# ielym/fastvision

Hardware: AMD Instinct MI355X
Metric: images/sec (640×640, bs=32/GPU) YOLOv3 train step, 1/2/4/8 MI355X (higher is better)
Workload: dtype bf16

## Files before the change

fastvision_amd/_lib.py:

```python
import ctypes as C
import os

HERE = os.path.dirname(os.path.abspath(__file__))
LIB_PATH = os.path.join(HERE, 'csrc', 'libfastvision_amd.so')
if os.environ.get('FVA_LIB_PATH'):
    if os.environ.get('FVA_EXPERIMENTS') == '1':
        LIB_PATH = os.environ['FVA_LIB_PATH']
        import sys
        print(f'fastvision_amd: EXPERIMENT -- loading {LIB_PATH} instead of the in-tree library (FVA_LIB_PATH)', file=sys.stderr)
    else:
        raise RuntimeError('fastvision_amd: FVA_LIB_PATH is set but FVA_EXPERIMENTS=1 is not -- refusing to load another library silently')

F32, BF16 = 0, 1


class ConvDesc(C.Structure):
    _fields_ = [(n, C.c_int32) for n in ('dtype', 'B', 'H', 'W', 'Cin', 'Cout', 'ksize', 'stride', 'in_pad', 'dy_pad')]


class HeadLevel(C.Structure):
    _fields_ = [('data', C.c_void_p), ('grad', C.c_void_p),
                ('sb', C.c_int64), ('sa', C.c_int64), ('sy', C.c_int64), ('sx', C.c_int64), ('sk', C.c_int64),
                ('B', C.c_int32), ('A', C.c_int32), ('H', C.c_int32), ('W', C.c_int32), ('K', C.c_int32),
                ('anchor_w', C.c_float * 8), ('anchor_h', C.c_float * 8), ('stride', C.c_float)]
# ... 53 lines not shown
    'fva_side_stream_renew': (_I, []),
    'fva_conv_debug_stamps': (_I, [_P, _I]),
    'fva_conv_patch_kernel': (_I, [_I]),
    'fva_profile_stop': (_I, [_P, _P, _P, _I]),
    'fva_conv_pack_weights': (_I, [_D, _P, _P, _P, _P]),
    'fva_conv_packed_elems': (_L, [_D, _I]),
    'fva_conv_pack_weights_multi': (_I, [_P, _I, _L, _P]),
    'fva_conv_pack_weights_tiled': (_I, [_P, _I, _I, _P]),
    'fva_conv_last_kernel': (C.c_char_p, []),
    'fva_conv_fwd': (_I, [_D, _P, _P, _P, _P, _P]),
    'fva_conv1x1_fwd_apply': (_I, [_D, _P, _P, _P, _P, _I, _P, _P, _P, _P, _P]),
    'fva_conv_fwd_acc': (_I, [_D, _P, _P, _P, _P, _I, _P]),
    'fva_bn_acc_finalize': (_I, [C.POINTER(BnFwdAcc), _L, _I, _P]),
    'fva_bn_silu_apply_acc': (_I, [_I, _P, C.POINTER(BnFwdAcc), _P, _I, _P, _I, _I, _I, _I, _I, _P]),
    'fva_conv1x1_fwd_apply_acc': (_I, [_D, _P, C.POINTER(BnFwdAcc), _P, _I, _P, _P, _P, _P, _I, _P]),
    'fva_conv_fwd_bnact': (_I, [_D, _P, _P, _P, _P, _P, _P, _I, _P]),
    'fva_conv_stat_blocks': (_I, [_D]),
    'fva_conv_dgrad': (_I, [_D, _P, _P, _P, _P, _P]),
    'fva_conv_dgrad_bnstats': (_I, [_D, _P, _P, _P, _P, C.POINTER(BnBwdFuse), _P]),
    'fva_conv_dgrad_stat_rows': (_I, [_D]),
    'fva_conv_wgrad': (_I, [_D, _P, _P, _P, _I, _P, _L, _P]),
    'fva_conv_wgrad_workspace': (_L, [_D]),
    'fva_conv_wgrad_plan': (_I, [_I]),
    'fva_stem_fwd': (_I, [_I, _P, _P, _P, _P, _P, _L, _I, _I, _I, _I, _I, _P]),
    'fva_stem_fwd_workspace': (_L, [_I, _I, _I, _I]),
    'fva_stem_stat_blocks': (_I, [_I, _I, _I, _I]),
    'fva_stem_fused_blocks': (_I, [_I, _I, _I]),
    'fva_stem_wgrad': (_I, [_I, _P, _P, _P, _I, _P, _L, _I, _I, _I, _I, _I, _P]),
    'fva_stem_wgrad_workspace': (_L, [_I, _I, _I, _I, _I]),
    'fva_stem_wgrad_mfma': (_I, [_P, _P, _P, _P, _L, _I, _I, _I, _P]),
    'fva_stem_wgrad_mfma_workspace': (_L, []),
    'fva_stem_pack': (_I, [_P, _P, _L, _I, _I, _I, _I, _P]),
    'fva_stem_fused': (_I, [_I, _P, _P, _P, _P, _P, _P, _P, _P, _P, _P, _I, _I, _I, _I, _P]),
    'fva_head_fwd': (_I, [_D, _P, _P, _P, _P, _P]),
    'fva_head_bwd_prepare': (_I, [_I, _P, _P, _P, _P, _I, _P, _I, _I, _I, _I, _I, _P]),
    'fva_bn_finalize': (_I, [_P, _I, _I, _L, _I, _P, _P, _P, _P, _P, _F, _F, _P, _P, _P, _P, _P]),
    'fva_bn_partial_rows': (_I, [_I]),
    'fva_bn_eval_coeffs': (_I, [_I, _P, _P, _P, _P, _F, _P, _P, _P]),
    'fva_bn_silu_apply': (_I, [_I, _P, _P, _P, _P, _I, _P, _I, _I, _I, _I, _I, _P]),
    'fva_bn_silu_bwd_reduce': (_I, [_I, _P, _P, _P, _P, _P, _P, _P, _I, _L, _I, _P]),
    'fva_bn_silu_bwd_reduce_acc': (_I, [_I, _P, _P, _P, _P, _P, _P, _P, _I, _L, _I, _P]),
    'fva_bn_bwd_blocks': (_I, [_I, _L, _I]),
    'fva_bn_bwd_finalize': (_I, [_P, _I, _I, _L, _I, _P, _P, _P, _P, _I, _P, _P]),
    'fva_bn_silu_bwd_apply': (_I, [_I, _P, _P, _P, _P, _P, _P, _P, _P, _I, _I, _I, _I, _I, _P]),
    'fva_bn_silu_bwd_apply_acc': (_I, [_I, _P, _P, _P, _P, _P, _P, C.POINTER(BnBwdAcc), _P, _I, _I, _I, _I, _I, _P]),
    'fva_upsample2_concat_fwd': (_I, [_I, _P, _I, _P, _I, _P, _I, _I, _I, _I, _I, _I, _P]),
    'fva_upsample2_concat_bwd': (_I, [_I, _P, _P, _P, _I, _I, _I, _I, _I, _I, _P]),
    'fva_pack_nchw': (_I, [_I, _P, _I, _L, _L, _L, _L, _P, _I, _I, _I, _I, _I, _P]),
    'fva_cast_nhwc': (_I, [_P, _I, _I, _P, _I, _I, _I, _I, _I, _I, _P]),
    'fva_yolov3_match': (_I, [_P, _I, _H, C.POINTER(MatchOut), _P]),
    'fva_yolov3_loss': (_I, [_P, _I, _H, _I, _F, _F, _F, _P, _P, _L, _P]),
    'fva_yolov3_loss_workspace': (_L, [_I, _H, _I]),
    'fva_yolov3_loss_dp': (_I, [_P, _I, _H, _I, _F, _F, _F, _P, _I, _P, _P, _L, _P]),
    'fva_scale_by_device_scalar': (_I, [_P, _L, _P, _P]),
    'fva_bce_loss': (_I, [_P, _P, _P, _P, _L, _L, _I, _I, _I, _P, _P, _P, _P]),
    'fva_row_loss': (_I, [_P, _P, _I, _I, _I, _F, _P, _P, _P, _P]),
    'fva_smooth_l1': (_I, [_P, _P, _L, _P, _P, _P, _P]),
    'fva_rows_relu_bwd_rows': (_I, [_I]),
    'fva_rows_relu_bwd': (_I, [_I, _P, _P, _P, _L, _P, _I, _I, _I, _P]),
    'fva_demo_loss': (_I, [_P, _I, _H, _I, _P, _P, _L, _P]),
    'fva_demo_loss_workspace': (_L, [_I, _H, _I]),
    'fva_demo_ciou_loss': (_I, [_P, _I, _H, _I, _P, _P, _L, _P]),
    'fva_demo_ciou_loss_workspace': (_L, [_I, _H, _I]),
    'fva_scale_head_groups': (_I, [_H, _P, _P, _P, _P]),
    'fva_iou_pairwise': (_I, [_I, _I, _I, _P, _P, _P, _P, _L, _F, _P]),
    'fva_iou_batch': (_I, [_I, _I, _I, _P, _P, _P, _L, _L, _F, _P]),
# ... 21 lines not shown
    'fva_colsum_scratch_rows': (_I, [_I]),
    'fva_colsum': (_I, [_P, _I, _I, _P, _P, _P]),
    'fva_maxpool2_fwd': (_I, [_I, _P, _I, _P, _I, _I, _I, _I, _I, _P]),
    'fva_maxpool2_bwd': (_I, [_I, _P, _P, _I, _P, _I, _I, _I, _I, _P]),
    'fva_rpn_decode': (_I, [_P, _P, _P, _P, _I, _I, _I, _I, _P]),
    'fva_rpn_match': (_I, [_P, _I, _P, _I, _I, _I, _I, _F, _F, _P, _P, _P]),
    'fva_fast_match': (_I, [_P, _I, _P, _I, _I, _F, _F, _F, _P, _P]),
    'fva_roi_align_fwd': (_I, [_I, _P, _I, _P, _I, _P, _I, _I, _I, _I, _I, _I, _F, _I, _P]),
    'fva_roi_align_bwd': (_I, [_P, _P, _I, _P, _I, _I, _I, _I, _I, _I, _F, _I, _P]),
    'fva_nms_select': (_I, [_P, _P, _I, _I, _I, C.POINTER(NmsParams), _P, _L, _P, _P, _P, _P]),
    'fva_gap_fwd': (_I, [_I, _P, _I, _I, _I, _I, _I, _P, _P]),
    'fva_gap_bwd': (_I, [_I, _P, _I, _I, _I, _I, _P, _P]),
    'fva_softmax_ce_workspace': (_L, [_I]),
    'fva_softmax_ce': (_I, [_P, _P, _I, _P, _I, _I, _I, _P, _P, _P, _P]),
    'fva_top1_accuracy': (_I, [_P, _I, _P, _I, _I, _I, _P, _P, _P]),
    'fva_bn_relu_apply': (_I, [_I, _P, _P, _P, _P, _I, _I, _I, _I, _I, _P]),
    'fva_bn_relu_bwd_reduce': (_I, [_I, _P, _P, _P, _P, _P, _P, _P, _I, _L, _I, _P]),
    'fva_bn_relu_bwd_apply': (_I, [_I, _P, _P, _P, _P, _P, _P, _P, _P, _I, _I, _I, _I, _I, _P]),
    'fva_bn_bias_running_mean': (_I, [_I, _P, _P, _F, _P]),
    'fva_bn_eval_coeffs_bias': (_I, [_I, _P, _P, _P, _P, _P, _F, _P, _P, _P]),
    'fva_adaptive_avgpool7_fwd': (_I, [_I, _P, _I, _I, _I, _I, _I, _P, _P]),
    'fva_adaptive_avgpool7_bwd': (_I, [_I, _P, _I, _I, _I, _I, _P, _P]),
    'fva_dropout_fwd': (_I, [_I, _P, _P, _L, _F, _P, _P]),
    'fva_dropout_bwd': (_I, [_I, _P, _P, _P, _L, _F, _P]),
    'fva_bn_frozen_bwd_blocks': (_I, [_I, _I, _I, _I, _I, _I]),
    'fva_bn_silu_frozen_bwd': (_I, [_I, _P, _P, _P, _P, _P, _P, _P, _P, _I, _I, _I, _I, _I, _P]),
    'fva_bn_relu_frozen_bwd': (_I, [_I, _P, _P, _P, _P, _P, _P, _P, _P, _I, _I, _I, _I, _I, _P]),
    'fva_bn_frozen_bwd_finalize': (_I, [_P, _I, _I, _I, _P, _P, _P, _P, _P]),
    'fva_bn_frozen_stats': (_I, [_I, _P, _P, _P, _F, _P, _P, _P]),
}
LABEL_I64, LABEL_F32 = 0, 1
REDUCE_MEAN, REDUCE_SUM = 0, 1
UNCHECKED = {'fva_conv_patch_kernel', 'fva_sgd_chunk_elems', 'fva_ema_chunk_elems', 'fva_rows_relu_bwd_rows', 'fva_colour_workspace', 'fva_conv_dgrad_stat_rows', 'fva_bias_relu_bwd_rows', 'fva_colsum_scratch_rows', 'fva_last_error', 'fva_version', 'fva_profile_stop', 'fva_conv_last_kernel', 'fva_conv_packed_elems', 'fva_conv_stat_blocks', 'fva_conv_wgrad_workspace', 'fva_conv_wgrad_plan',
             'fva_stem_stat_blocks', 'fva_stem_fused_blocks', 'fva_stem_wgrad_workspace', 'fva_stem_fwd_workspace', 'fva_stem_wgrad_mfma_workspace', 'fva_bn_bwd_blocks', 'fva_bn_partial_rows', 'fva_yolov3_loss_workspace',
             'fva_demo_loss_workspace', 'fva_demo_ciou_loss_workspace', 'fva_nms_candidates_workspace', 'fva_nms_select_workspace', 'fva_softmax_ce_workspace', 'fva_bn_frozen_bwd_blocks'}

_lib = None


def load():
    global _lib
    if _lib is not None:
        return _lib
    if not os.path.exists(LIB_PATH):
        raise RuntimeError(f'fastvision_amd: {LIB_PATH} is missing -- the HIP extension is REQUIRED (no CPU fallback). '
                           'Build it with `python fastvision_amd/csrc/build.py`.')
    lib = C.CDLL(LIB_PATH)
    for name, (res, args) in PROTOTYPES.items():
        fn = getattr(lib, name)
        fn.restype, fn.argtypes = res, args
    _lib = lib
    return lib


tracer = None


_fns = {}


def call(name, *args):
    fn = _fns.get(name)
    if fn is None:
        fn = _fns[name] = getattr(load(), name)
    lib = _lib
    if tracer is not None:
        span = tracer(name, args)
# ... 11 lines not shown
```

fastvision_amd/csrc/errors.hip:

```cpp
#include "common.h"
thread_local char fva_err_buf[512] = "";
extern "C" const char* fva_last_error(void) { return fva_err_buf; }
extern "C" int fva_version(void) { return 7; }
static thread_local const char* g_last_kernel = "";
void fva_note_kernel(const char* name) { g_last_kernel = name; }
extern "C" const char* fva_conv_last_kernel(void) { return g_last_kernel; }

#include <vector>
namespace {
struct Span { hipEvent_t e0, e1; int cls; double flop; };
std::vector<Span> g_spans;
int g_used = 0;
bool g_on = false;
unsigned g_mask = ~0u;
int g_stride = 1, g_seen = 0;
}

FvaProfileSpan::FvaProfileSpan(int cls, double flop, hipStream_t s) : slot(-1), stream(s) {
    if (!g_on || !((g_mask >> (cls & 0xff)) & 1u) || (g_seen++ % g_stride) != 0 || g_used >= (int)g_spans.size()) return;
    slot = g_used++;
    g_spans[slot].cls = cls;
    g_spans[slot].flop = flop;
    (void)hipEventRecord(g_spans[slot].e0, stream);
}
FvaProfileSpan::~FvaProfileSpan() {
    if (slot >= 0) (void)hipEventRecord(g_spans[slot].e1, stream);
}

extern "C" int fva_profile_start(int32_t max_spans) {
    if (max_spans < 0) return fva_fail(FVA_ERR_ARG, "fva_profile_start: negative span count");
    while ((int)g_spans.size() < max_spans) {
        Span sp{};
        if (hipEventCreate(&sp.e0) != hipSuccess || hipEventCreate(&sp.e1) != hipSuccess) return fva_fail(FVA_ERR_LAUNCH, "fva_profile_start: hipEventCreate failed");
        (void)hipEventRecord(sp.e0, nullptr);
        (void)hipEventRecord(sp.e1, nullptr);
        g_spans.push_back(sp);
// ... 123 lines not shown
```

fastvision_amd/csrc/stem.hip:

```cpp
#include <stdlib.h>

#include "common.h"

namespace {

constexpr int CO = 32;
constexpr int MAXJ = 36;

template <typename T>
__global__ __launch_bounds__(256) void stem_fwd_kernel(const float* __restrict__ img, const float* __restrict__ w,
                                                       T* __restrict__ y, float* __restrict__ stats, int B, int Cin, int H,
                                                       int W, int64_t M) {
    __shared__ float sw[MAXJ * CO];
    __shared__ float tile[256 * 33];
    const int tid = threadIdx.x;
    const int J = Cin * 9;
    for (int i = tid; i < J * CO; i += 256) {
        const int co = i % CO, j = i / CO;
        sw[j * CO + co] = w[co * J + j];
    }
    __syncthreads();
    const int64_t m = (int64_t)blockIdx.x * 256 + tid;
    const bool live = m < M;
    float acc[CO];
#pragma unroll
    for (int c = 0; c < CO; ++c) acc[c] = 0.f;
    if (live) {
        const int x = (int)(m % W), yy = (int)((m / W) % H), b = (int)(m / ((int64_t)W * H));
#pragma unroll 1
        for (int ci = 0; ci < Cin; ++ci) {
            const float* plane = img + ((int64_t)b * Cin + ci) * H * W;
#pragma unroll 1
            for (int kh = 0; kh < 3; ++kh)
// ... 218 lines not shown
        for (int c = 0; c < 2; ++c) {
            bf16x4 o;
#pragma unroll
            for (int j = 0; j < 4; ++j) {
                o[j] = (bf16_t)acc[c][j];
                s1[c][j] += acc[c][j];
                s2[c][j] += acc[c][j] * acc[c][j];
            }
            *(bf16x4*)(yo + 16 * c) = o;
        }
    }
    if (stats == nullptr) return;
#pragma unroll
    for (int c = 0; c < 2; ++c)
#pragma unroll
        for (int j = 0; j < 4; ++j) {
#pragma unroll
            for (int o = 1; o < 16; o <<= 1) {
                s1[c][j] += __shfl_xor(s1[c][j], o);
                s2[c][j] += __shfl_xor(s2[c][j], o);
            }
            if (r == 0) {
                red[0][wv][16 * c + 4 * g + j] = s1[c][j];
                red[1][wv][16 * c + 4 * g + j] = s2[c][j];
            }
        }
    __syncthreads();
    if (tid < 64) {
        const int which = tid >> 5, ch = tid & 31;
        stats[((int64_t)blockIdx.x * 2 + which) * 32 + ch] = (red[which][0][ch] + red[which][1][ch]) + (red[which][2][ch] + red[which][3][ch]);
    }
}

enum { STEM_STATS = 0, STEM_APPLY = 1, STEM_REDUCE = 2, STEM_DGRAD = 3 };

struct StemFusedParams {
    const uint2* img4;
    const float* w;
    const bf16_t* dz;
    const float *scale, *shift, *mean, *rstd, *coef;
    bf16_t* out;
    float* part;
    int Cin, H, W;
    int64_t M;
};

template <int MODE>
__global__ __launch_bounds__(256) void stem_fused_kernel(const StemFusedParams p) {
    __shared__ float red[2][4][32];
    const int tid = threadIdx.x, lane = tid & 63, wv = tid >> 6;
    const int r = lane & 15, g = lane >> 4;
    const int H = p.H, W = p.W, Wp = W + 2;
    __shared__ float wsh[CO * 27];
    bf16x8 wa[2][2];
    stem_weight_fragments<true>(p.w, p.Cin, wsh, wa);
    const int ta = 2 * g, tb = 2 * g + 1;
    const int offa = (ta / 3) * Wp + ta % 3, offb = (tb / 3) * Wp + tb % 3, offc = 2 * Wp + 2;
    float sc[2][4], sh[2][4], mu[2][4], rs[2][4], ka[2][4], k1[2][4], k2[2][4], s1[2][4], s2[2][4];
#pragma unroll
    for (int c = 0; c < 2; ++c)
#pragma unroll
        for (int j = 0; j < 4; ++j) {
            const int ch = 8 * g + 4 * c + j;
            s1[c][j] = s2[c][j] = 0.f;
            if constexpr (MODE != STEM_STATS) {
                sc[c][j] = p.scale[ch];
                sh[c][j] = p.shift[ch];
            }
            if constexpr (MODE == STEM_REDUCE || MODE == STEM_DGRAD) {
                mu[c][j] = p.mean[ch];
                rs[c][j] = p.rstd[ch];
            }
            if constexpr (MODE == STEM_DGRAD) {
                ka[c][j] = p.coef[ch];
                k1[c][j] = p.coef[32 + ch] * rs[c][j];
                k2[c][j] = p.coef[64 + ch] - k1[c][j] * mu[c][j];
            }
        }

    constexpr int STEM_NB = MODE == STEM_REDUCE ? 2 : 4;
    const int tiles_per_row = W / 16;
    const int nchunks = (int)((p.M / 16 + STEM_TPW - 1) / STEM_TPW);
    const int wvu = __builtin_amdgcn_readfirstlane(wv);
    for (int chunk = blockIdx.x * 4 + wvu; chunk < nchunks; chunk += gridDim.x * 4) {
    const int tile0 = chunk * STEM_TPW;
    int64_t m0 = (int64_t)tile0 * 16;
    const int row0 = tile0 / tiles_per_row;
    int x0 = (tile0 - row0 * tiles_per_row) * 16;
    const int b0 = row0 / H;
    int yy = row0 - b0 * H;
    int64_t hpix = ((int64_t)b0 * (H + 2) + yy) * Wp + x0;
    for (int bt = 0; bt < STEM_TPW / STEM_NB; ++bt) {
    uint2 la[STEM_NB], lb[STEM_NB], lc[STEM_NB];
    bf16x8 gz[STEM_NB];
    int64_t hp[STEM_NB];
    bool ok[STEM_NB];
#pragma unroll
    for (int i = 0; i < STEM_NB; ++i) {
        ok[i] = m0 < p.M;
        hp[i] = hpix + r;
        if (ok[i]) {
            const uint2* base = p.img4 + hp[i];
            la[i] = base[offa];
            lb[i] = base[offb];
            lc[i] = base[offc];
            if constexpr (MODE == STEM_REDUCE || MODE == STEM_DGRAD) gz[i] = *(const bf16x8*)(p.dz + (m0 + r) * 32 + 8 * g);
        }
        m0 += 16;
        x0 += 16;
        hpix += 16;
        if (x0 == W) {
// ... 36 lines not shown
                    const float du = (float)gzc[4 * c + j] * silu_grad(yv * sc[c][j] + sh[c][j]);
                    if constexpr (MODE == STEM_REDUCE) {
                        s1[c][j] += du;
                        s2[c][j] += du * (yv - mu[c][j]) * rs[c][j];
                    } else {
                        o[4 * c + j] = (bf16_t)(ka[c][j] * du + k1[c][j] * yv + k2[c][j]);
                    }
                }
            }
        }
        if constexpr (MODE == STEM_APPLY || MODE == STEM_DGRAD) *(bf16x8*)oo = o;
    }
    }
    }
    if constexpr (MODE == STEM_STATS || MODE == STEM_REDUCE) {
#pragma unroll
        for (int c = 0; c < 2; ++c)
#pragma unroll
            for (int j = 0; j < 4; ++j) {
#pragma unroll
                for (int o = 1; o < 16; o <<= 1) {
                    s1[c][j] += __shfl_xor(s1[c][j], o);
                    s2[c][j] += __shfl_xor(s2[c][j], o);
                }
                if (r == 0) {
                    red[0][wv][8 * g + 4 * c + j] = s1[c][j];
                    red[1][wv][8 * g + 4 * c + j] = s2[c][j];
                }
            }
        __syncthreads();
        if (tid < 64) {
            const int which = tid >> 5, ch = tid & 31;
            p.part[((int64_t)blockIdx.x * 2 + which) * 32 + ch] = (red[which][0][ch] + red[which][1][ch]) + (red[which][2][ch] + red[which][3][ch]);
        }
    }
}

constexpr int WGRAD_BLOCKS = 1024;
constexpr int STEM_FUSED_GRID = 2048;

}

extern "C" {

static bool stem_mfma(int dtype, int W) {
    static const bool on = [] { const char* e = getenv("FVA_STEM_MFMA"); return !e || atoi(e) != 0; }();
    return on && dtype == FVA_BF16 && W % 16 == 0;
}

int32_t fva_stem_stat_blocks(int dtype, int B, int H, int W) {
    const int64_t M = (int64_t)B * H * W;
    return stem_mfma(dtype, W) ? cdiv(M, STEM_BLOCK_PIX) : cdiv(M, 256);
}

int64_t fva_stem_fwd_workspace(int dtype, int B, int H, int W) {
    return stem_mfma(dtype, W) ? (int64_t)B * (H + 2) * (W + 2) * 8 + 64 : 0;
}

int fva_stem_fwd(int dtype, const float* img, const float* w, void* y, float* stats, void* workspace, int64_t workspace_bytes, int B,
                 int Cin, int H, int W, int Cout, void* stream) {
    if (!img || !w || !y) return fva_fail(FVA_ERR_ARG, "fva_stem_fwd: null pointer");
    if (Cout != CO || Cin < 1 || Cin > 3) return fva_fail(FVA_ERR_ARG, "fva_stem_fwd: needs Cout==32, Cin<=3 (got %d, %d)", Cout, Cin);
    const int64_t M = (int64_t)B * H * W;
    const int grid = cdiv(M, 256);
    hipStream_t s = (hipStream_t)stream;
    if (stem_mfma(dtype, W)) {
// ... 58 lines not shown
    hipLaunchKernelGGL(stem_pack_kernel, dim3((int)((hp + 255) / 256 < 65536 ? (hp + 255) / 256 : 65536)), dim3(256), 0, (hipStream_t)stream, img,
                       (uint2*)img4, B, Cin, H, W);
    FVA_LAUNCH_CHECK("stem_pack_kernel");
    return FVA_OK;
}

int fva_stem_fused(int mode, const void* img4, const float* w, const void* dz, const float* scale, const float* shift, const float* mean,
                   const float* rstd, const float* coef, void* out, float* part, int B, int Cin, int H, int W, void* stream) {
    if (!img4 || !w || Cin < 1 || Cin > 3 || W % 16) return fva_fail(FVA_ERR_ARG, "fva_stem_fused: bad argument");
    const bool need_affine = mode != STEM_STATS, need_dz = mode == STEM_REDUCE || mode == STEM_DGRAD;
    if ((need_affine && (!scale || !shift)) || (need_dz && (!dz || !mean || !rstd)) || (mode == STEM_DGRAD && !coef) ||
        ((mode == STEM_APPLY || mode == STEM_DGRAD) && !out) || ((mode == STEM_STATS || mode == STEM_REDUCE) && !part))
        return fva_fail(FVA_ERR_ARG, "fva_stem_fused: missing operand for mode %d", mode);
    StemFusedParams p{};
    p.img4 = (const uint2*)img4; p.w = w; p.dz = (const bf16_t*)dz;
    p.scale = scale; p.shift = shift; p.mean = mean; p.rstd = rstd; p.coef = coef;
    p.out = (bf16_t*)out; p.part = part;
    p.Cin = Cin; p.H = H; p.W = W; p.M = (int64_t)B * H * W;
    if (p.M / 16 > INT32_MAX) return fva_fail(FVA_ERR_ARG, "fva_stem_fused: batch of %lld pixels too large", (long long)p.M);
    const dim3 grid(fva_stem_fused_blocks(B, H, W));
    hipStream_t s = (hipStream_t)stream;
    switch (mode) {
        case STEM_STATS: hipLaunchKernelGGL(stem_fused_kernel<STEM_STATS>, grid, dim3(256), 0, s, p); break;
        case STEM_APPLY: hipLaunchKernelGGL(stem_fused_kernel<STEM_APPLY>, grid, dim3(256), 0, s, p); break;
        case STEM_REDUCE: hipLaunchKernelGGL(stem_fused_kernel<STEM_REDUCE>, grid, dim3(256), 0, s, p); break;
        case STEM_DGRAD: hipLaunchKernelGGL(stem_fused_kernel<STEM_DGRAD>, grid, dim3(256), 0, s, p); break;
        default: return fva_fail(FVA_ERR_ARG, "fva_stem_fused: bad mode %d", mode);
    }
    FVA_LAUNCH_CHECK("stem_fused_kernel");
    if (mode == STEM_APPLY || mode == STEM_DGRAD) return fva_zero_halo_border(out, B, H, W, 4, 1, s);
    return FVA_OK;
}

}
```

fastvision_amd/ops.py:

```python
import ctypes as C
import os
import weakref
import threading

import torch

from . import _lib
from ._lib import BF16, F32, ConvDesc

_state = threading.local()
_default_dtype = torch.bfloat16


def set_compute_dtype(dtype):
    global _default_dtype
    if dtype not in (torch.bfloat16, torch.float32):
        raise ValueError('compute dtype must be torch.bfloat16 or torch.float32')
    _default_dtype = dtype


def get_compute_dtype():
    return getattr(_state, 'dtype', None) or _default_dtype


# ... 681 lines not shown

    @staticmethod
    def forward(ctx, x, weight, gamma, beta, bn, training, stride, dtype):
        require_gpu(x, 'ConvBlock')
        keep, x_ptr, x_pad = to_halo(x, dtype, weight.shape[2] // 2)
        need = _GRAD_ON[0] and any(ctx.needs_input_grad)
        z, s = conv_block_fwd(x, x_ptr, x_pad, weight, gamma, beta, bn, training, stride, dtype, need_ctx=need, may_defer=True)
        if s is not None:
            s.keep = keep
        ctx.s = s
        ctx.x_like = x
        return z

    @staticmethod
    def backward(ctx, dz):
        s = ctx.s
        if s is None:
            raise _released('ConvBlock')
        keep, dz_ptr = to_dense(dz, s.dtype)
        dx, dw, dg, db = conv_block_bwd(s, dz_ptr, ctx.needs_input_grad[0], needs=ctx.needs_input_grad[1:4])
        x_like, ctx.s, ctx.x_like = ctx.x_like, None, None
        return (_grad_like(dx, x_like) if dx is not None else None), dw, dg, db, None, None, None, None


def _stem_wgrad_mfma(img4, dy, B, Cin, H, W, Cout):
    lib, dev = _lib.load(), dy.device
    raw = torch.empty((Cout, 4, 4, 3), dtype=torch.float32, device=dev)
    wsb = lib.fva_stem_wgrad_mfma_workspace()
    ws = torch.empty(wsb, dtype=torch.uint8, device=dev)
    _lib.call('fva_stem_wgrad_mfma', _p(img4), _p(dy), _p(raw), _p(ws), wsb, B, H, W, _stream())
    return raw[:, :3, :Cin, :].permute(0, 2, 3, 1).contiguous()


def _stem_wgrad_direct(code, img, dy, wshape, B, Cin, H, W, Cout):
    lib, dev = _lib.load(), dy.device
    dw = torch.empty(wshape, dtype=torch.float32, device=dev)
    wsb = lib.fva_stem_wgrad_workspace(B, Cin, H, W, Cout)
    ws = torch.empty(wsb, dtype=torch.uint8, device=dev)
    _lib.call('fva_stem_wgrad', code, _p(img), _p(dy), _p(dw), 0, _p(ws), wsb, B, Cin, H, W, Cout, _stream())
    return dw


class StemFn(torch.autograd.Function):

    @staticmethod
    def forward(ctx, images, weight, gamma, beta, bn, training, dtype):
        require_gpu(images, 'stem')
        flush_pending_apply()
        img = images.detach()
        if img.dtype != torch.float32 or not img.is_contiguous():
            img = img.float().contiguous()
        B, Cin, H, W = img.shape
        Cout = weight.shape[0]
        lib = _lib.load()
        dev, code = img.device, _code(dtype)
        M = B * H * W
        scale = torch.empty(Cout, dtype=torch.float32, device=dev)
        shift = torch.empty_like(scale)
        mean = rstd = None
        wsb = lib.fva_stem_fwd_workspace(code, B, H, W)
        ws = torch.empty(wsb, dtype=torch.uint8, device=dev) if wsb else None
        frozen = not training and _GRAD_ON[0] and any(ctx.needs_input_grad)
        ctx.bn = bn if frozen else None
        if ws is not None and os.environ.get('FVA_STEM_FUSED', '1') != '0' and not frozen:
            _lib.call('fva_stem_pack', _p(img), _p(ws), wsb, B, Cin, H, W, _stream())
            if training:
# ... 25 lines not shown
        zbuf, z = halo_alloc(B, Cout, H, W, dtype, dev, 1)
        _lib.call('fva_bn_silu_apply', code, _p(y), _p(scale), _p(shift), C.c_void_p(0), 0, _p(zbuf), 1, B, H, W, Cout, _stream())
        ctx.saved = (img, y, scale, shift, mean, rstd, gamma, dtype, training, tuple(weight.shape))
        ctx.img4 = ws
        return z

    @staticmethod
    def backward(ctx, dz):
        if ctx.saved is None:
            raise _released('stem')
        img, y, scale, shift, mean, rstd, gamma, dtype, training, wshape = ctx.saved
        img4, w_saved = ctx.img4, getattr(ctx, 'weight', None)
        bn, ctx.bn = getattr(ctx, 'bn', None), None
        ctx.saved = ctx.img4 = ctx.weight = None
        if ctx.needs_input_grad[0]:
            raise RuntimeError('fastvision_amd: the stem does not produce a gradient for the input images')
        lib = _lib.load()
        B, Cin, H, W = img.shape
        Cout, code, dev = wshape[0], _code(dtype), img.device
        M = B * H * W
        keep, dz_ptr = to_dense(dz, dtype)
        if y is None and not training:
            raise RuntimeError('fastvision_amd: the stem ran its fused inference path (gradients were off in forward): nothing was saved for backward')
        if y is None:
            w = w_saved
            nb = lib.fva_stem_fused_blocks(B, H, W)
            part = torch.empty((lib.fva_bn_partial_rows(nb), 2, Cout), dtype=torch.float32, device=dev)
            _lib.call('fva_stem_fused', 2, _p(img4), _p(w), C.c_void_p(dz_ptr), _p(scale), _p(shift), _p(mean), _p(rstd), None, None,
                      _p(part), B, Cin, H, W, _stream())
            dgamma = torch.empty(Cout, dtype=torch.float32, device=dev)
            dbeta = torch.empty_like(dgamma)
            coef = torch.empty((3, Cout), dtype=torch.float32, device=dev)
            _lib.call('fva_bn_bwd_finalize', _p(part), nb, part.shape[0], M, Cout, _p(gamma), _p(rstd), _p(dgamma), _p(dbeta), 0, _p(coef), _stream())
            dy = torch.empty((B, H + 2, W + 2, Cout), dtype=dtype, device=dev)
            _lib.call('fva_stem_fused', 3, _p(img4), _p(w), C.c_void_p(dz_ptr), _p(scale), _p(shift), _p(mean), _p(rstd), _p(coef),
                      _p(dy), None, B, Cin, H, W, _stream())
            return None, _stem_wgrad_mfma(img4, dy, B, Cin, H, W, Cout), dgamma, dbeta, None, None, None
        mfma = img4 is not None and os.environ.get('FVA_STEM_WGRAD_MFMA', '1') != '0'
        if not training:
            need_w, need_g, need_b = ctx.needs_input_grad[1:4]
            dy = torch.empty((B, H + 2, W + 2, Cout) if mfma else (M, Cout), dtype=dtype, device=dev)
            dgamma, dbeta, _ = frozen_bn_bwd('silu', code, dz_ptr, y, scale, shift, bn, None, dy, 1 if mfma else 0, B, H, W, Cout, need_g, need_b)
            dw = None
            if need_w:
                dw = _stem_wgrad_mfma(img4, dy, B, Cin, H, W, Cout) if mfma else _stem_wgrad_direct(code, img, dy, wshape, B, Cin, H, W, Cout)
            return None, dw, dgamma, dbeta, None, None, None
        nb = lib.fva_bn_bwd_blocks(code, M, Cout)
        part = torch.empty((lib.fva_bn_partial_rows(nb), 2, Cout), dtype=torch.float32, device=dev)
        _lib.call('fva_bn_silu_bwd_reduce', code, C.c_void_p(dz_ptr), _p(y), _p(scale), _p(shift), _p(mean), _p(rstd), _p(part),
                  nb, M, Cout, _stream())
        dgamma = torch.empty(Cout, dtype=torch.float32, device=dev)
        dbeta = torch.empty_like(dgamma)
        coef = torch.empty((3, Cout), dtype=torch.float32, device=dev)
        _lib.call('fva_bn_bwd_finalize', _p(part), nb, part.shape[0], M, Cout, _p(gamma), _p(rstd), _p(dgamma), _p(dbeta), 0, _p(coef), _stream())
        if mfma:
            dy = torch.empty((B, H + 2, W + 2, Cout), dtype=dtype, device=dev)
            _lib.call('fva_bn_silu_bwd_apply', code, C.c_void_p(dz_ptr), _p(y), _p(scale), _p(shift), _p(mean), _p(rstd), _p(coef),
                      _p(dy), 1, B, H, W, Cout, _stream())
            return None, _stem_wgrad_mfma(img4, dy, B, Cin, H, W, Cout), dgamma, dbeta, None, None, None
        dy = torch.empty((M, Cout), dtype=dtype, device=dev)
        _lib.call('fva_bn_silu_bwd_apply', code, C.c_void_p(dz_ptr), _p(y), _p(scale), _p(shift), _p(mean), _p(rstd), _p(coef),
                  _p(dy), 0, B, H, W, Cout, _stream())
        return None, _stem_wgrad_direct(code, img, dy, wshape, B, Cin, H, W, Cout), dgamma, dbeta, None, None, None


class ResidualFn(torch.autograd.Function):
# ... 172 lines not shown
```

include/fastvision_amd.h:

```cpp
#ifndef FASTVISION_AMD_H
#define FASTVISION_AMD_H

#include <stdint.h>

#ifdef __cplusplus
extern "C" {
#endif

typedef enum { FVA_F32 = 0, FVA_BF16 = 1 } fva_dtype;

typedef enum {
    FVA_OK = 0,
    FVA_ERR_ARG = -1,
    FVA_ERR_LAUNCH = -2,
    FVA_ERR_WORKSPACE = -3
} fva_status;

const char* fva_last_error(void);
int fva_version(void);

int fva_profile_start(int32_t max_spans);
int fva_profile_classes(uint32_t mask, int32_t stride);

int fva_side_stream_fork(void* main_stream, void** side_stream);
// ... 38 lines not shown
int fva_conv_dgrad(const fva_conv_desc* d, const void* dy, const void* w_dgrad, void* dx, const void* addend, void* stream);

typedef struct {
    const void* y;
    const float *scale, *shift, *mean, *rstd;
    float* partial;
    int64_t* acc;
    int32_t acc_replicas;
} fva_bn_bwd_fuse;
int fva_conv_dgrad_bnstats(const fva_conv_desc* d, const void* dy, const void* w_dgrad, void* dx, const void* addend,
                           const fva_bn_bwd_fuse* fuse, void* stream);
int32_t fva_conv_dgrad_stat_rows(const fva_conv_desc* d);

int fva_conv_wgrad(const fva_conv_desc* d, const void* x, const void* dy, float* dw_oihw, int accumulate,
                   void* workspace, int64_t workspace_bytes, void* stream);
int64_t fva_conv_wgrad_workspace(const fva_conv_desc* d);
int fva_conv_wgrad_plan(int beside);

int fva_stem_fwd(int dtype, const float* images_nchw, const float* w_oihw, void* y, float* stats_partial,
                 void* workspace, int64_t workspace_bytes, int B, int Cin, int H, int W, int Cout, void* stream);
int64_t fva_stem_fwd_workspace(int dtype, int B, int H, int W);
int32_t fva_stem_stat_blocks(int dtype, int B, int H, int W);
int32_t fva_stem_fused_blocks(int B, int H, int W);
int fva_stem_wgrad(int dtype, const float* images_nchw, const void* dy, float* dw_oihw, int accumulate,
                   void* workspace, int64_t workspace_bytes, int B, int Cin, int H, int W, int Cout, void* stream);
int64_t fva_stem_wgrad_workspace(int B, int Cin, int H, int W, int Cout);
int fva_stem_wgrad_mfma(const void* images_nhwc4, const void* dy_halo, float* dw_raw, void* workspace, int64_t workspace_bytes,
                        int B, int H, int W, void* stream);
int64_t fva_stem_wgrad_mfma_workspace(void);
int fva_stem_pack(const float* images_nchw, void* images_nhwc4, int64_t bytes, int B, int Cin, int H, int W, void* stream);
int fva_stem_fused(int mode, const void* images_nhwc4, const float* w_oihw, const void* dz, const float* scale, const float* shift,
                   const float* save_mean, const float* save_rstd, const float* coef, void* out, float* part, int B, int Cin, int H,
                   int W, void* stream);

int fva_head_fwd(const fva_conv_desc* d, const void* x, const void* w_fwd, const float* bias, float* out, void* stream);
int fva_head_bwd_prepare(int dtype, const float* dhead, const float* grad_scale, void* dy, float* dbias,
                         int accumulate, void* workspace, int B, int H, int W, int N, int Npad, void* stream);

int32_t fva_bn_partial_rows(int32_t nblocks);
int fva_bn_finalize(float* stats_partial, int32_t nblocks, int32_t partial_rows, int64_t count, int32_t C,
                    const float* gamma, const float* beta, float* running_mean, float* running_var,
                    int64_t* num_batches_tracked, float momentum, float eps, float* save_mean, float* save_rstd,
                    float* scale, float* shift, void* stream);
int fva_bn_eval_coeffs(int32_t C, const float* gamma, const float* beta, const float* running_mean,
                       const float* running_var, float eps, float* scale, float* shift, void* stream);
int fva_bn_silu_apply(int dtype, const void* y, const float* scale, const float* shift, const void* residual,
                      int res_pad, void* z, int z_pad, int B, int H, int W, int C, void* stream);
#define FVA_BN_ACC_WORDS 5
#define FVA_BN_ACC_MAX_REPLICAS 32
typedef struct {
    int64_t* acc;
    int64_t* zero;
    int32_t replicas;
    const float *gamma, *beta;
    float *running_mean, *running_var;
    int64_t* num_batches_tracked;
    float momentum, eps;
    float *save_mean, *save_rstd, *scale, *shift;
} fva_bn_fwd_acc;
typedef struct {
    int64_t* acc;
    int64_t* zero;
    int32_t replicas;
    const float* gamma;
    float *dgamma, *dbeta;
    int32_t accumulate;
// ... 220 lines not shown
```

Before: 1131.

## Fuse stem BN-SiLU backward with weight-gradient MFMA, skipping dy materialization

Adds a STEM_WGRAD mode to the fused stem kernel. It recomputes the conv output, applies the BN+SiLU backward in registers, and stages dy and image patches in double-buffered LDS. It then accumulates the weight gradient with MFMA, using transposed LDS reads (ds_read_b64_tr_b16) and a split-K slab, followed by a small reduce kernel. This avoids writing and re-reading a full-resolution padded dy tensor at 640x640 for the stem wgrad. The cost is a split-K workspace, an extra reduce launch, and tricky LDS layout code. It is enabled by default through an environment flag.

```diff
diff --git a/fastvision_amd/_lib.py b/fastvision_amd/_lib.py
--- a/fastvision_amd/_lib.py
+++ b/fastvision_amd/_lib.py
@@ -109,6 +109,8 @@
     'fva_stem_wgrad_mfma_workspace': (_L, []),
     'fva_stem_pack': (_I, [_P, _P, _L, _I, _I, _I, _I, _P]),
     'fva_stem_fused': (_I, [_I, _P, _P, _P, _P, _P, _P, _P, _P, _P, _P, _I, _I, _I, _I, _P]),
+    'fva_stem_fused_wgrad': (_I, [_P, _P, _P, _P, _P, _P, _P, _P, _P, _P, _L, _I, _I, _I, _I, _P]),
+    'fva_stem_fused_wgrad_workspace': (_L, []),
     'fva_head_fwd': (_I, [_D, _P, _P, _P, _P, _P]),
     'fva_head_bwd_prepare': (_I, [_I, _P, _P, _P, _P, _I, _P, _I, _I, _I, _I, _I, _P]),
     'fva_bn_finalize': (_I, [_P, _I, _I, _L, _I, _P, _P, _P, _P, _P, _F, _F, _P, _P, _P, _P, _P]),
@@ -196,7 +198,7 @@
 LABEL_I64, LABEL_F32 = 0, 1
 REDUCE_MEAN, REDUCE_SUM = 0, 1
 UNCHECKED = {'fva_conv_patch_kernel', 'fva_sgd_chunk_elems', 'fva_ema_chunk_elems', 'fva_rows_relu_bwd_rows', 'fva_colour_workspace', 'fva_conv_dgrad_stat_rows', 'fva_bias_relu_bwd_rows', 'fva_colsum_scratch_rows', 'fva_last_error', 'fva_version', 'fva_profile_stop', 'fva_conv_last_kernel', 'fva_conv_packed_elems', 'fva_conv_stat_blocks', 'fva_conv_wgrad_workspace', 'fva_conv_wgrad_plan',
-             'fva_stem_stat_blocks', 'fva_stem_fused_blocks', 'fva_stem_wgrad_workspace', 'fva_stem_fwd_workspace', 'fva_stem_wgrad_mfma_workspace', 'fva_bn_bwd_blocks', 'fva_bn_partial_rows', 'fva_yolov3_loss_workspace',
+             'fva_stem_stat_blocks', 'fva_stem_fused_blocks', 'fva_stem_wgrad_workspace', 'fva_stem_fwd_workspace', 'fva_stem_wgrad_mfma_workspace', 'fva_stem_fused_wgrad_workspace', 'fva_bn_bwd_blocks', 'fva_bn_partial_rows', 'fva_yolov3_loss_workspace',
              'fva_demo_loss_workspace', 'fva_demo_ciou_loss_workspace', 'fva_nms_candidates_workspace', 'fva_nms_select_workspace', 'fva_softmax_ce_workspace', 'fva_bn_frozen_bwd_blocks'}
 
 _lib = None
diff --git a/fastvision_amd/csrc/errors.hip b/fastvision_amd/csrc/errors.hip
--- a/fastvision_amd/csrc/errors.hip
+++ b/fastvision_amd/csrc/errors.hip
@@ -1,7 +1,7 @@
 #include "common.h"
 thread_local char fva_err_buf[512] = "";
 extern "C" const char* fva_last_error(void) { return fva_err_buf; }
-extern "C" int fva_version(void) { return 7; }
+extern "C" int fva_version(void) { return 8; }
 static thread_local const char* g_last_kernel = "";
 void fva_note_kernel(const char* name) { g_last_kernel = name; }
 extern "C" const char* fva_conv_last_kernel(void) { return g_last_kernel; }
diff --git a/fastvision_amd/csrc/stem.hip b/fastvision_amd/csrc/stem.hip
--- a/fastvision_amd/csrc/stem.hip
+++ b/fastvision_amd/csrc/stem.hip
@@ -1,4 +1,6 @@
 #include <stdlib.h>
+
+#include <type_traits>
 
 #include "common.h"
 
@@ -283,7 +285,24 @@
     }
 }
 
-enum { STEM_STATS = 0, STEM_APPLY = 1, STEM_REDUCE = 2, STEM_DGRAD = 3 };
+enum { STEM_STATS = 0, STEM_APPLY = 1, STEM_REDUCE = 2, STEM_DGRAD = 3, STEM_WGRAD = 4 };
+
+constexpr int WG_PIX = 128, WG_DY = 80, WG_P = 72;
+constexpr int WG_POFF = WG_PIX * WG_DY;
+constexpr int WG_IMG = WG_PIX * (WG_DY + WG_P);
+constexpr int WG_SLOTS = 32, WG_ROW = WG_SLOTS * CO;
+constexpr int WG_KSPLIT = 512;
+
+template <int OFF>
+__device__ __forceinline__ s16x4 stem_tr_read(uint32_t addr) {
+    s16x4 v;
+    asm volatile("ds_read_b64_tr_b16 %0, %1 offset:%2" : "=v"(v) : "v"(addr), "n"(OFF) : "memory");
+    return v;
+}
+using s16x8 = __attribute__((ext_vector_type(8))) short;
+__device__ __forceinline__ bf16x8 stem_cat8(s16x4 lo, s16x4 hi) {
+    return __builtin_bit_cast(bf16x8, (s16x8)__builtin_shufflevector(lo, hi, 0, 1, 2, 3, 4, 5, 6, 7));
+}
 
 struct StemFusedParams {
     const uint2* img4;
@@ -292,6 +311,8 @@
     const float *scale, *shift, *mean, *rstd, *coef;
     bf16_t* out;
     float* part;
+    float* slab;
+    int mchunk;
     int Cin, H, W;
     int64_t M;
 };
@@ -318,16 +339,125 @@
                 sc[c][j] = p.scale[ch];
                 sh[c][j] = p.shift[ch];
             }
-            if constexpr (MODE == STEM_REDUCE || MODE == STEM_DGRAD) {
+            if constexpr (MODE == STEM_REDUCE || MODE == STEM_DGRAD || MODE == STEM_WGRAD) {
                 mu[c][j] = p.mean[ch];
                 rs[c][j] = p.rstd[ch];
             }
-            if constexpr (MODE == STEM_DGRAD) {
+            if constexpr (MODE == STEM_DGRAD || MODE == STEM_WGRAD) {
                 ka[c][j] = p.coef[ch];
                 k1[c][j] = p.coef[32 + ch] * rs[c][j];
                 k2[c][j] = p.coef[64 + ch] - k1[c][j] * mu[c][j];
             }
         }
+
+    if constexpr (MODE == STEM_WGRAD) {
+    __shared__ __attribute__((aligned(16))) char wst[2 * WG_IMG];
+    const int wvu = __builtin_amdgcn_readfirstlane(wv);
+    const int kt = wvu >> 1, ct = wvu & 1;
+    const int tiles_per_row = W / 16;
+    const int tbeg = (int)((int64_t)blockIdx.x * p.mchunk / 16);
+    const int64_t mlast = (int64_t)(blockIdx.x + 1) * p.mchunk;
+    const int tend = (int)((mlast < p.M ? mlast : p.M) / 16);
+    const int nsteps = (tend - tbeg + 7) / 8;
+    const uint32_t wtr = (uint32_t)(size_t)LDS_PTR(wst) + (uint32_t)((8 * g + (r >> 2)) * WG_DY + 8 * (r & 3) + 32 * ct);
+    const uint32_t wtp = (uint32_t)(size_t)LDS_PTR(wst) + (uint32_t)(WG_POFF + (8 * g + (r >> 2)) * WG_P + 8 * (r & 3) + 32 * kt);
+    for (int i = tid; i < 2 * WG_PIX; i += 256)
+        *(uint2*)(wst + (i >> 7) * WG_IMG + WG_POFF + (i & 127) * WG_P + 56) = make_uint2(0u, 0u);
+    f32x4 dwa = f32x4{0.f, 0.f, 0.f, 0.f};
+    uint2 la[2][2], lb[2][2], lc[2][2];
+    bf16x8 gz[2][2];
+    bool ok[2][2];
+    auto issue = [&](int step, auto stage_tag) {
+        constexpr int S = decltype(stage_tag)::value;
+#pragma unroll
+        for (int i = 0; i < 2; ++i) {
+            const int t = tbeg + step * 8 + 2 * wvu + i;
+            ok[S][i] = t < tend;
+            if (ok[S][i]) {
+                const int row = t / tiles_per_row;
+                const int x0 = (t - row * tiles_per_row) * 16;
+                const int b = row / H, yy = row - b * H;
+                const uint2* base = p.img4 + (((int64_t)b * (H + 2) + yy) * Wp + x0 + r);
+                la[S][i] = base[offa];
+                lb[S][i] = base[offb];
+                lc[S][i] = base[offc];
+                gz[S][i] = *(const bf16x8*)(p.dz + ((int64_t)t * 16 + r) * 32 + 8 * g);
+            }
+        }
+    };
+    auto body = [&](int step, auto stage_tag) {
+        constexpr int S = decltype(stage_tag)::value;
+        if (step + 1 < nsteps) issue(step + 1, std::integral_constant<int, S ^ 1>{});
+        char* img = wst + S * WG_IMG;
+#pragma unroll
+        for (int i = 0; i < 2; ++i) {
+            char* drow = img + (32 * wv + 16 * i + r) * WG_DY + 16 * g;
+            char* prow = img + WG_POFF + (32 * wv + 16 * i + r) * WG_P;
+            uint32_t* pd = (uint32_t*)(prow + 12 * g);
+            if (!ok[S][i]) {
+                *(uint4*)drow = make_uint4(0u, 0u, 0u, 0u);
+                pd[0] = pd[1] = pd[2] = 0u;
+                if (g == 0) *(uint2*)(prow + 48) = make_uint2(0u, 0u);
+                continue;
+            }
+            const uint2 ta4 = la[S][i], tb4 = lb[S][i], tc4 = lc[S][i];
+            const bf16x8 p0 = __builtin_bit_cast(bf16x8, make_uint4(ta4.x, ta4.y, tb4.x, tb4.y));
+            const bf16x8 p1 = __builtin_bit_cast(bf16x8, g == 0 ? make_uint4(tc4.x, tc4.y, 0u, 0u) : make_uint4(0u, 0u, 0u, 0u));
+            const bf16x8 gzc = gz[S][i];
+            f32x4 acc[2];
+#pragma unroll
+            for (int c = 0; c < 2; ++c) {
+                acc[c] = f32x4{0.f, 0.f, 0.f, 0.f};
+                acc[c] = __builtin_amdgcn_mfma_f32_16x16x32_bf16(wa[c][0], p0, acc[c], 0, 0, 0);
+                acc[c] = __builtin_amdgcn_mfma_f32_16x16x32_bf16(wa[c][1], p1, acc[c], 0, 0, 0);
+            }
+            bf16x8 o;
+#pragma unroll
+            for (int c = 0; c < 2; ++c)
+#pragma unroll
+                for (int j = 0; j < 4; ++j) {
+                    const float yv = acc[c][j];
+                    const float du = (float)gzc[4 * c + j] * silu_grad(yv * sc[c][j] + sh[c][j]);
+                    o[4 * c + j] = (bf16_t)(ka[c][j] * du + k1[c][j] * yv + k2[c][j]);
+                }
+            *(bf16x8*)drow = o;
+            pd[0] = ta4.x;
+            pd[1] = (ta4.y & 0xffffu) | (tb4.x << 16);
+            pd[2] = (tb4.x >> 16) | (tb4.y << 16);
+            if (g == 0) *(uint2*)(prow + 48) = tc4;
+        }
+        __syncthreads();
+        constexpr int O = S * WG_IMG;
+        s16x4 a0 = stem_tr_read<O>(wtp), a1 = stem_tr_read<O + 4 * WG_P>(wtp);
+        s16x4 b0 = stem_tr_read<O>(wtr), b1 = stem_tr_read<O + 4 * WG_DY>(wtr);
+        s16x4 a2 = stem_tr_read<O + 32 * WG_P>(wtp), a3 = stem_tr_read<O + 36 * WG_P>(wtp);
+        s16x4 b2 = stem_tr_read<O + 32 * WG_DY>(wtr), b3 = stem_tr_read<O + 36 * WG_DY>(wtr);
+        s16x4 a4 = stem_tr_read<O + 64 * WG_P>(wtp), a5 = stem_tr_read<O + 68 * WG_P>(wtp);
+        s16x4 b4 = stem_tr_read<O + 64 * WG_DY>(wtr), b5 = stem_tr_read<O + 68 * WG_DY>(wtr);
+        s16x4 a6 = stem_tr_read<O + 96 * WG_P>(wtp), a7 = stem_tr_read<O + 100 * WG_P>(wtp);
+        s16x4 b6 = stem_tr_read<O + 96 * WG_DY>(wtr), b7 = stem_tr_read<O + 100 * WG_DY>(wtr);
+        asm volatile("s_waitcnt lgkmcnt(0)"
+                     : "+v"(a0), "+v"(a1), "+v"(a2), "+v"(a3), "+v"(a4), "+v"(a5), "+v"(a6), "+v"(a7), "+v"(b0), "+v"(b1), "+v"(b2), "+v"(b3),
+                       "+v"(b4), "+v"(b5), "+v"(b6), "+v"(b7)
+                     :
+                     : "memory");
+        __builtin_amdgcn_sched_barrier(0);
+        dwa = __builtin_amdgcn_mfma_f32_16x16x32_bf16(stem_cat8(a0, a1), stem_cat8(b0, b1), dwa, 0, 0, 0);
+        dwa = __builtin_amdgcn_mfma_f32_16x16x32_bf16(stem_cat8(a2, a3), stem_cat8(b2, b3), dwa, 0, 0, 0);
+        dwa = __builtin_amdgcn_mfma_f32_16x16x32_bf16(stem_cat8(a4, a5), stem_cat8(b4, b5), dwa, 0, 0, 0);
+        dwa = __builtin_amdgcn_mfma_f32_16x16x32_bf16(stem_cat8(a6, a7), stem_cat8(b6, b7), dwa, 0, 0, 0);
+    };
+    __syncthreads();
+    if (nsteps > 0) issue(0, std::integral_constant<int, 0>{});
+    for (int step = 0; step < nsteps; step += 2) {
+        body(step, std::integral_constant<int, 0>{});
+        if (step + 1 < nsteps) body(step + 1, std::integral_constant<int, 1>{});
+    }
+    float* row = p.slab + (int64_t)blockIdx.x * WG_ROW;
+#pragma unroll
+    for (int j = 0; j < 4; ++j) row[(16 * kt + 4 * g + j) * CO + 16 * ct + r] = dwa[j];
+    return;
+    }
 
     constexpr int STEM_NB = MODE == STEM_REDUCE ? 2 : 4;
     const int tiles_per_row = W / 16;
@@ -430,6 +560,37 @@
         if (tid < 64) {
             const int which = tid >> 5, ch = tid & 31;
             p.part[((int64_t)blockIdx.x * 2 + which) * 32 + ch] = (red[which][0][ch] + red[which][1][ch]) + (red[which][2][ch] + red[which][3][ch]);
+        }
+    }
+}
+
+__global__ __launch_bounds__(256) void stem_fused_wgrad_reduce_kernel(const float* __restrict__ slab, float* __restrict__ raw, int ksplit) {
+    __shared__ float part[4][64];
+    if (blockIdx.x == WG_ROW / 64) {
+        for (int e = threadIdx.x; e < CO * 48; e += 256) {
+            const int q = e % 48, kw = q / 12, ci = (q / 3) & 3;
+            if (kw == 3 || ci == 3) raw[e] = 0.f;
+        }
+        return;
+    }
+    const int li = threadIdx.x & 63, grp = threadIdx.x >> 6;
+    const int e = blockIdx.x * 64 + li;
+    const float* src = slab + e;
+    float s = 0.f;
+    int k = grp;
+    for (; k + 12 < ksplit; k += 16) {
+        const float v0 = src[(int64_t)k * WG_ROW], v1 = src[(int64_t)(k + 4) * WG_ROW];
+        const float v2 = src[(int64_t)(k + 8) * WG_ROW], v3 = src[(int64_t)(k + 12) * WG_ROW];
+        s += (v0 + v1) + (v2 + v3);
+    }
+    for (; k < ksplit; k += 4) s += src[(int64_t)k * WG_ROW];
+    part[grp][li] = s;
+    __syncthreads();
+    if (grp == 0) {
+        const int slot = e / CO, co = e - slot * CO;
+        if (slot < 27) {
+            const int tap = slot / 3, ci = slot - 3 * tap, kh = tap / 3, kw = tap - 3 * kh;
+            raw[co * 48 + kw * 12 + ci * 3 + kh] = (part[0][li] + part[1][li]) + (part[2][li] + part[3][li]);
         }
     }
 }
@@ -554,4 +715,32 @@
     return FVA_OK;
 }
 
-}
+int64_t fva_stem_fused_wgrad_workspace(void) { return (int64_t)WG_KSPLIT * WG_ROW * 4; }
+
+int fva_stem_fused_wgrad(const void* img4, const float* w, const void* dz, const float* scale, const float* shift, const float* mean,
+                         const float* rstd, const float* coef, float* dw_raw, void* workspace, int64_t workspace_bytes, int B, int Cin,
+                         int H, int W, void* stream) {
+    if (!img4 || !w || !dz || !scale || !shift || !mean || !rstd || !coef || !dw_raw || !workspace)
+        return fva_fail(FVA_ERR_ARG, "fva_stem_fused_wgrad: null pointer");
+    if (Cin < 1 || Cin > 3 || W % 16 || B < 1 || H < 1 || W < 1) return fva_fail(FVA_ERR_ARG, "fva_stem_fused_wgrad: bad argument");
+    const int64_t M = (int64_t)B * H * W;
+    if (M >= (1ll << 31)) return fva_fail(FVA_ERR_ARG, "fva_stem_fused_wgrad: batch of %lld pixels too large", (long long)M);
+    const int mchunk = cdiv(cdiv(M, WG_KSPLIT), 64) * 64;
+    const int ksplit = cdiv(M, mchunk);
+    const int64_t need = (int64_t)ksplit * WG_ROW * 4;
+    if (workspace_bytes < need) return fva_fail(FVA_ERR_WORKSPACE, "fva_stem_fused_wgrad: workspace %lld < %lld", (long long)workspace_bytes, (long long)need);
+    StemFusedParams p{};
+    p.img4 = (const uint2*)img4; p.w = w; p.dz = (const bf16_t*)dz;
+    p.scale = scale; p.shift = shift; p.mean = mean; p.rstd = rstd; p.coef = coef;
+    p.slab = (float*)workspace; p.mchunk = mchunk;
+    p.Cin = Cin; p.H = H; p.W = W; p.M = M;
+    hipStream_t s = (hipStream_t)stream;
+    FvaProfileSpan span(2 | (3 << 8), 2.0 * p.M * 32.0 * 27.0, s);
+    hipLaunchKernelGGL(stem_fused_kernel<STEM_WGRAD>, dim3(ksplit), dim3(256), 0, s, p);
+    FVA_LAUNCH_CHECK("stem_fused_kernel");
+    hipLaunchKernelGGL(stem_fused_wgrad_reduce_kernel, dim3(WG_ROW / 64 + 1), dim3(256), 0, s, (const float*)workspace, dw_raw, ksplit);
+    FVA_LAUNCH_CHECK("stem_fused_wgrad_reduce_kernel");
+    return FVA_OK;
+}
+
+}
diff --git a/fastvision_amd/ops.py b/fastvision_amd/ops.py
--- a/fastvision_amd/ops.py
+++ b/fastvision_amd/ops.py
@@ -737,6 +737,19 @@
     return raw[:, :3, :Cin, :].permute(0, 2, 3, 1).contiguous()
 
 
+_STEM_FUSED_WGRAD = [os.environ.get('FVA_STEM_FUSED_WGRAD', '1') != '0']
+
+
+def _stem_fused_wgrad(img4, w, dz_ptr, scale, shift, mean, rstd, coef, B, Cin, H, W, Cout):
+    lib, dev = _lib.load(), img4.device
+    raw = torch.empty((Cout, 4, 4, 3), dtype=torch.float32, device=dev)
+    wsb = lib.fva_stem_fused_wgrad_workspace()
+    ws = torch.empty(wsb, dtype=torch.uint8, device=dev)
+    _lib.call('fva_stem_fused_wgrad', _p(img4), _p(w), C.c_void_p(dz_ptr), _p(scale), _p(shift), _p(mean), _p(rstd), _p(coef), _p(raw), _p(ws),
+              wsb, B, Cin, H, W, _stream())
+    return raw[:, :3, :Cin, :].permute(0, 2, 3, 1).contiguous()
+
+
 def _stem_wgrad_direct(code, img, dy, wshape, B, Cin, H, W, Cout):
     lib, dev = _lib.load(), dy.device
     dw = torch.empty(wshape, dtype=torch.float32, device=dev)
@@ -828,6 +841,9 @@
             dbeta = torch.empty_like(dgamma)
             coef = torch.empty((3, Cout), dtype=torch.float32, device=dev)
             _lib.call('fva_bn_bwd_finalize', _p(part), nb, part.shape[0], M, Cout, _p(gamma), _p(rstd), _p(dgamma), _p(dbeta), 0, _p(coef), _stream())
+            if _STEM_FUSED_WGRAD[0]:
+                dw = _stem_fused_wgrad(img4, w, dz_ptr, scale, shift, mean, rstd, coef, B, Cin, H, W, Cout)
+                return None, dw, dgamma, dbeta, None, None, None
             dy = torch.empty((B, H + 2, W + 2, Cout), dtype=dtype, device=dev)
             _lib.call('fva_stem_fused', 3, _p(img4), _p(w), C.c_void_p(dz_ptr), _p(scale), _p(shift), _p(mean), _p(rstd), _p(coef),
                       _p(dy), None, B, Cin, H, W, _stream())
diff --git a/include/fastvision_amd.h b/include/fastvision_amd.h
--- a/include/fastvision_amd.h
+++ b/include/fastvision_amd.h
@@ -94,6 +94,10 @@
 int fva_stem_fused(int mode, const void* images_nhwc4, const float* w_oihw, const void* dz, const float* scale, const float* shift,
                    const float* save_mean, const float* save_rstd, const float* coef, void* out, float* part, int B, int Cin, int H,
                    int W, void* stream);
+int fva_stem_fused_wgrad(const void* images_nhwc4, const float* w_oihw, const void* dz, const float* scale, const float* shift,
+                         const float* save_mean, const float* save_rstd, const float* coef, float* dw_raw, void* workspace,
+                         int64_t workspace_bytes, int B, int Cin, int H, int W, void* stream);
+int64_t fva_stem_fused_wgrad_workspace(void);
 
 int fva_head_fwd(const fva_conv_desc* d, const void* x, const void* w_fwd, const float* bias, float* out, void* stream);
 int fva_head_bwd_prepare(int dtype, const float* dhead, const float* grad_scale, void* dy, float* dbias,
```

New measurement: 1142 (median of 4 runs). 1.01x the previous value.
